# nfurnon/disco

Measured on NVIDIA H100. Metric: beamformed frames/sec (16kHz, 512-pt STFT), higher is better.
Workload: dtype f32 (c64 spectra, f32 SCM accumulation, f64 per-bin solve)

## Files before the change

### disco_b200/_lib.py

```python
import ctypes
import os

_HERE = os.path.dirname(os.path.abspath(__file__))
LIB_PATH = os.path.join(_HERE, "libdisco_b200.so")

c_int, c_void_p, c_size_t, c_float, c_double = (ctypes.c_int, ctypes.c_void_p, ctypes.c_size_t,
                                                ctypes.c_float, ctypes.c_double)
c_int_p = ctypes.POINTER(ctypes.c_int)

SIGNATURES = {
    "disco_abi_version": (c_int, []),
    "disco_last_error": (ctypes.c_char_p, []),
    "disco_n_frames": (c_int, [c_int, c_int]),
    "disco_init": (c_int, [c_int]),
    "disco_set_reserved_sms": (c_int, [c_int]),
    "disco_stft": (c_int, [c_void_p, c_void_p, c_int, c_int, c_int, c_void_p]),
    "disco_stft_scm_workspace": (c_size_t, [c_int, c_int, c_int, c_int]),
    "disco_stft_scm": (c_int, [c_void_p, c_void_p, c_int, c_void_p, c_void_p, c_void_p, c_int, c_int, c_int, c_int,
                               c_void_p, c_size_t, c_void_p]),
    "disco_stft_scm_supported": (c_int, [c_int, c_int, c_int]),
    "disco_stft_scm2_workspace": (c_size_t, [c_int, c_int, c_int, c_int]),
    "disco_stft_scm2": (c_int, [c_void_p, c_void_p, c_void_p, c_int, c_void_p, c_int, c_int, c_int, c_int, c_void_p,
                                c_size_t, c_void_p]),
    "disco_stft_filter_dual": (c_int, [c_void_p, c_void_p, c_void_p, c_void_p, c_void_p, c_void_p, c_int, c_int, c_int,
                                       c_int, c_int, c_int, c_void_p]),
    "disco_scm_from_workspace": (c_int, [c_void_p, c_int, c_int, c_void_p, c_void_p, c_int, c_int, c_int, c_int,
                                         c_void_p]),
    "disco_mwf_solve_workspace2": (c_int, [c_void_p, c_void_p, c_void_p, c_int, c_int, c_int, c_int, c_int, c_int,
                                           c_double, c_void_p]),
    "disco_filter_dual": (c_int, [c_void_p, c_void_p, c_void_p, c_void_p, c_void_p, c_void_p, c_int, c_int, c_int,
                                  c_int, c_int, c_int, c_void_p]),
    "disco_tf_mask": (c_int, [c_void_p, c_void_p, c_void_p, c_size_t, c_int, c_int, c_float, c_void_p]),
    "disco_masked_scm": (c_int, [c_void_p, c_void_p, c_void_p, c_int, c_void_p, c_void_p, c_int, c_int, c_int, c_int,
                                 c_int, c_int_p, c_int, c_int, c_void_p]),
    "disco_filter_sum_scm": (c_int, [c_void_p, c_void_p, c_void_p, c_int, c_void_p, c_void_p, c_int, c_void_p, c_void_p,
                                     c_int, c_int, c_int, c_int, c_void_p]),
    "disco_tango_mid_supported": (c_int, [c_int, c_int]),
    "disco_tango_mid": (c_int, [c_void_p, c_void_p, c_void_p, c_void_p, c_void_p, c_int, c_void_p, c_void_p, c_int, c_int,
                                c_int, c_int, c_int, c_void_p]),
    "disco_mwf_solve_workspace": (c_int, [c_void_p, c_void_p, c_void_p, c_void_p, c_void_p, c_int, c_int, c_int, c_int,
                                          c_int, c_int, c_double, c_void_p]),
    "disco_mwf_solve": (c_int, [c_void_p, c_void_p, c_void_p, c_void_p, c_int, c_int, c_int, c_int, c_double,
                                c_void_p]),
    "disco_filter_sum": (c_int, [c_void_p, c_int, c_void_p, c_void_p, c_void_p, c_void_p, c_int, c_int, c_int, c_int,
                                 c_int, c_int, c_int, c_int_p, c_int, c_int, c_void_p]),
    "disco_istft": (c_int, [c_void_p, c_void_p, c_int, c_int, c_int, c_int, c_void_p]),
    "disco_scm_recursive": (c_int, [c_void_p, c_void_p, c_void_p, c_void_p, c_void_p, c_void_p, c_void_p, ctypes.c_double,
                                    c_int, c_int, c_int, c_int, c_int, c_int, c_int, c_int_p, c_int, c_void_p]),
    "disco_filter_sum_blocks": (c_int, [c_void_p, c_int, c_void_p, c_void_p, c_void_p, c_void_p, c_int, c_int, c_int,
                                        c_int, c_int, c_int, c_int, c_int, c_int_p, c_int, c_void_p]),
    "disco_band_stats": (c_int, [c_void_p, c_void_p, c_void_p, c_void_p, c_int, c_int, ctypes.c_longlong, c_int, c_int,
                                 c_void_p]),
    "disco_transpose_c64": (c_int, [c_void_p, c_void_p, c_int, c_int, c_int, c_void_p]),
    "disco_transpose_f32": (c_int, [c_void_p, c_void_p, c_int, c_int, c_int, c_void_p]),
    "disco_apply_mask": (c_int, [c_void_p, c_void_p, c_void_p, c_size_t, c_int, c_void_p]),
    "disco_apply_mask_channels": (c_int, [c_void_p, c_void_p, c_void_p, c_size_t, c_int, c_size_t, c_int, c_void_p]),
}

_lib = None


def load():
    global _lib
    if _lib is not None:
        return _lib
    if not os.path.exists(LIB_PATH):
        raise ImportError(
            "disco_b200: %s not found -- build the CUDA library first (python -m disco_b200.build). "
            "There is no CPU or PyTorch fallback." % LIB_PATH)
    lib = ctypes.CDLL(LIB_PATH)
    for name, (res, args) in SIGNATURES.items():
        fn = getattr(lib, name)
        fn.restype = res
        fn.argtypes = args
    if lib.disco_abi_version() != 2:
        raise ImportError("disco_b200: ABI version mismatch")
    _lib = lib
    return lib


class DiscoError(RuntimeError):
    pass


def check(rc):
    if rc != 0:
        msg = load().disco_last_error()
        raise DiscoError("libdisco_b200 error %d: %s" % (rc, msg.decode() if msg else "?"))
```

### disco_b200/build.py

```python
import os
import subprocess
import sys
from concurrent.futures import ThreadPoolExecutor

HERE = os.path.dirname(os.path.abspath(__file__))
ROOT = os.path.dirname(HERE)
CSRC = os.path.join(HERE, "csrc")
OBJ = os.path.join(ROOT, "build", "obj")
LIB = os.path.join(HERE, "libdisco_b200.so")
SOURCES = ["api.cu", "stft_scm.cu", "scm.cu", "scm_wide.cu", "solve.cu", "solve_small.cu", "filter_sum.cu", "filter_sum_multi.cu", "filter_dual.cu", "mid_multi.cu", "istft.cu", "filterbank.cu", "online.cu", "misc.cu"]
NVCC = os.environ.get("NVCC", "/usr/local/cuda/bin/nvcc")
FLAGS = ["-O3", "-std=c++17", "-gencode", "arch=compute_90a,code=sm_90a", "-lineinfo",
         "-Xcompiler", "-fPIC", "-Xcompiler", "-fvisibility=hidden"]


def _deps_mtime():
    newest = 0.0
    for dirpath in (CSRC, os.path.join(ROOT, "include")):
        for fn in os.listdir(dirpath):
            if fn.endswith((".cuh", ".h")):
                newest = max(newest, os.path.getmtime(os.path.join(dirpath, fn)))
    return newest


def build(verbose=False, force=False):
    os.makedirs(OBJ, exist_ok=True)
    hdr = _deps_mtime()
    jobs = []
    for src in SOURCES:
        s = os.path.join(CSRC, src)
        o = os.path.join(OBJ, src.replace(".cu", ".o"))
        if force or not os.path.exists(o) or os.path.getmtime(o) < max(os.path.getmtime(s), hdr):
            cmd = [NVCC] + FLAGS + (["-Xptxas", "-v"] if verbose else []) + ["-c", s, "-o", o]
            jobs.append(cmd)

    def run(cmd):
        r = subprocess.run(cmd, capture_output=True, text=True)
        return cmd, r

    with ThreadPoolExecutor(max_workers=min(8, max(1, len(jobs)))) as ex:
        for cmd, r in ex.map(run, jobs):
            if verbose or r.returncode != 0:
                sys.stderr.write(" ".join(cmd) + "\n" + r.stdout + r.stderr + "\n")
            if r.returncode != 0:
                raise RuntimeError("nvcc failed for %s" % cmd[-3])
    objs = [os.path.join(OBJ, s.replace(".cu", ".o")) for s in SOURCES]
    if force or jobs or not os.path.exists(LIB):
        cmd = [NVCC, "-shared", "-o", LIB] + objs + ["-gencode", "arch=compute_90a,code=sm_90a"]
        r = subprocess.run(cmd, capture_output=True, text=True)
        if r.returncode != 0:
            sys.stderr.write(r.stdout + r.stderr)
            raise RuntimeError("link failed")
    return LIB


if __name__ == "__main__":
    print(build(verbose="-v" in sys.argv, force="--force" in sys.argv))
```

### disco_b200/csrc/stft_scm.cu

```cuda
#include "common.cuh"
#include "fft_reg.cuh"
#include "kernels.h"

namespace disco {

enum : int { OUT_Y = 0, OUT_NONE = 1, OUT_FILTER = 2, OUT_FILTER_FT = 3 };

template <int N, int C, int NM = 1, int OUT = OUT_Y>
struct StftCfg {
    static constexpr int RA = N / 32;
    static constexpr int NB = 32 / RA;
    static constexpr int HALF = N / 2;
    static constexpr int F = N / 2 + 1;
    static constexpr bool WIDE = C > 4;
    static constexpr int NSTG = 2;
    static constexpr int JOBS = 8;
    static constexpr int ITEMS = JOBS * NB;
    static constexpr int P = (C + 1) / 2;
    static constexpr int TT = ITEMS / P;
    static constexpr bool REALLOC = (N == 512) || (WIDE && N == 256);
    static constexpr int FFT_WARPS = (N == 512 && (WIDE || NM == 2)) ? 4 : 8;
    static constexpr int JPW = JOBS / FFT_WARPS;
    static constexpr int ROWP = 1056 / NB;
    static constexpr int SCM_WARPS = N / 64;
    static constexpr int LEAD_WARPS = REALLOC ? 4 : 1;
    static constexpr int WARPS = LEAD_WARPS + FFT_WARPS + SCM_WARPS;
    static constexpr int THREADS = 32 * WARPS;
    static constexpr int SPEC = ITEMS * ROWP;
    static constexpr int SAMP = C * (TT + 1) * HALF;
    static constexpr int REG_LAUNCH = 16384 / ((WARPS + 3) / 4) / 32 / 8 * 8;
    static constexpr bool FILT = OUT == OUT_FILTER || OUT == OUT_FILTER_FT;
    static constexpr int REG_LEAD = FILT ? 56 : 32;
    static constexpr int REG_SCM = FILT ? 80 : WIDE ? 184 : (FFT_WARPS == 4 ? 152 : 120);
    static constexpr int REG_FFT_CAP = 256;
    static constexpr int REG_ALLOC = (REG_LAUNCH > 255 ? 255 : REG_LAUNCH) * THREADS;
    static constexpr int REG_FFT_LEFT = (REG_ALLOC - 128 * REG_LEAD - 32 * SCM_WARPS * REG_SCM) / (32 * FFT_WARPS) / 8 * 8;
    static constexpr int REG_FFT = REG_FFT_LEFT < REG_FFT_CAP ? REG_FFT_LEFT : REG_FFT_CAP;
    static constexpr int REG_SUM = 128 * REG_LEAD + 32 * FFT_WARPS * REG_FFT + 32 * SCM_WARPS * REG_SCM;
    static constexpr int FT_PITCH = 34;
    static constexpr int FT_STAGE = OUT == OUT_FILTER_FT ? SCM_WARPS * 8 * FT_PITCH : 0;
    static_assert(!REALLOC || (REG_LEAD >= 24 && REG_FFT >= 24), "setmaxnreg budgets start at 24");
    static_assert(!REALLOC || REG_SUM <= (REG_LAUNCH > 255 ? 255 : REG_LAUNCH) * THREADS,
                  "register budgets exceed the CTA's allocation");
};

int stft_tile_frames(int n_fft, int C) { return (8 * (32 / (n_fft / 32))) / ((C + 1) / 2); }

template <int N, int C, int OUT = OUT_Y>
__host__ __device__ inline size_t smem_bytes() {
    using G = StftCfg<N, C, 1, OUT>;
    return G::NSTG * ((size_t)G::SPEC * sizeof(float2) + (size_t)G::SAMP * sizeof(float)) + (size_t)N * sizeof(float2) + 256 +
           64 * sizeof(float) + (size_t)G::FT_STAGE * sizeof(float2);
}

__device__ __forceinline__ long long range_lo(long long total, int b, int nb) { return total * b / nb; }

template <int R, int LAUNCH>
DISCO_DEV void set_maxnreg() {
    if constexpr (R > LAUNCH) {
        asm volatile("setmaxnreg.inc.sync.aligned.u32 %0;\n" ::"n"(R));
    } else if constexpr (R < LAUNCH) {
        asm volatile("setmaxnreg.dec.sync.aligned.u32 %0;\n" ::"n"(R));
    }
}

template <int C, int NM>
struct ScmAcc {
    static constexpr int NOFF = C * (C - 1) / 2;
    static constexpr int NO = NOFF > 0 ? NOFF : 1;
    float2 d[NM > 0 ? NM : 1][C];
    float2 os[NM > 0 ? NM : 1][NO];
    float2 on[NM > 0 ? NM : 1][NO];
    DISCO_DEV void reset() {
#pragma unroll
        for (int q = 0; q < NM; ++q) {
#pragma unroll
            for (int i = 0; i < C; ++i) d[q][i] = make_float2(0.f, 0.f);
#pragma unroll
            for (int i = 0; i < NOFF; ++i) os[q][i] = on[q][i] = make_float2(0.f, 0.f);
        }
    }
    DISCO_DEV void step(const float2 (&y)[C], const float (&m)[NM > 0 ? NM : 1]) {
        float2 ab[NM > 0 ? NM : 1];
#pragma unroll
        for (int q = 0; q < NM; ++q) {
            const float om = 1.f - m[q];
            ab[q] = make_float2(m[q] * m[q], om * om);
        }
        int o = 0;
#pragma unroll
        for (int i = 0; i < C; ++i) {
            const float dd = fmaf(y[i].x, y[i].x, y[i].y * y[i].y);
#pragma unroll
            for (int q = 0; q < NM; ++q) d[q][i] = ffma2(make_float2(dd, dd), ab[q], d[q][i]);
#pragma unroll
            for (int j = i + 1; j < C; ++j) {
                const float2 op = cmulc(y[i], y[j]);
#pragma unroll
                for (int q = 0; q < NM; ++q) {
                    os[q][o] = cfma_r(ab[q].x, op, os[q][o]);
                    on[q][o] = cfma_r(ab[q].y, op, on[q][o]);
                }
                ++o;
            }
        }
    }
    DISCO_DEV void flush(float* out, int F) const {
        int a = 0;
#pragma unroll
        for (int q = 0; q < NM; ++q) {
#pragma unroll
            for (int i = 0; i < C; ++i) out[(size_t)(a++) * F] = d[q][i].x;
#pragma unroll
            for (int i = 0; i < NOFF; ++i) {
                out[(size_t)(a++) * F] = os[q][i].x;
                out[(size_t)(a++) * F] = os[q][i].y;
            }
#pragma unroll
            for (int i = 0; i < C; ++i) out[(size_t)(a++) * F] = d[q][i].y;
#pragma unroll
            for (int i = 0; i < NOFF; ++i) {
                out[(size_t)(a++) * F] = on[q][i].x;
                out[(size_t)(a++) * F] = on[q][i].y;
            }
        }
    }
};

template <int OUT>
struct StftParam {
    using type = StftArgs;
};
template <>
struct StftParam<OUT_FILTER> {
    using type = StftFilterArgs;
};
template <>
struct StftParam<OUT_FILTER_FT> {
    using type = StftFilterArgs;
};

template <int N, int C, int NM, int OUT>
__global__ void __launch_bounds__(StftCfg<N, C, NM, OUT>::THREADS, 1) stft_scm_kernel(typename StftParam<OUT>::type p) {
    using G = StftCfg<N, C, NM, OUT>;
    constexpr int RA = G::RA, NB = G::NB, H = G::HALF, F = G::F, ROWP = G::ROWP, P = G::P, TT = G::TT;
    constexpr int SAMP = G::SAMP;
    constexpr int NACC = NM * 2 * C * C;
    constexpr int NMX = NM > 0 ? NM : 1;
    constexpr bool SCM = NM > 0;
    constexpr bool STORE_Y = OUT == OUT_Y, FILT = G::FILT, FT = OUT == OUT_FILTER_FT;
    static_assert(!FILT || NM == 0, "the filter consumer accumulates no statistics");
    constexpr int MCAP = (G::REALLOC && G::REG_SCM >= 152 && !G::WIDE) ? 16 : 8;
    constexpr int MC = (TT * NM <= MCAP) ? TT : ((MCAP / NMX) < TT ? (MCAP / NMX) : TT);
    constexpr int NCH = (TT + MC - 1) / MC;

    extern __shared__ __align__(128) unsigned char smem_raw[];
    constexpr int NSTG = G::NSTG;
    float2* spec = reinterpret_cast<float2*>(smem_raw);
    float* samp = reinterpret_cast<float*>(spec + NSTG * G::SPEC);
    float2* tw = reinterpret_cast<float2*>(samp + NSTG * SAMP);
    uint64_t* bars = reinterpret_cast<uint64_t*>(tw + N);
    uint64_t* samp_full = bars;
    uint64_t* samp_empty = bars + NSTG;
    uint64_t* spec_full = bars + 2 * NSTG;
    uint64_t* spec_empty = bars + 3 * NSTG;
    float* nyq = reinterpret_cast<float*>(bars + 32);
    float2* ft_stage = reinterpret_cast<float2*>(nyq + 64);
    static_assert(4 * NSTG <= 32, "barrier area");
    static_assert(TT * C <= 64 && TT <= 32, "Nyquist staging");

    const int tid = threadIdx.x, lane = tid & 31, warp = tid >> 5;
    const int L = p.L, T = p.T;
    const int tiles_per_grp = (T + TT - 1) / TT;
    const long long total = (long long)p.n_grp * tiles_per_grp;
    const long long lo = range_lo(total, blockIdx.x, gridDim.x), hi = range_lo(total, blockIdx.x + 1, gridDim.x);
    const int n_it = (int)(hi - lo);
    if (n_it <= 0) return;

    for (int i = tid; i < N; i += blockDim.x) tw[i] = p.twiddle[i];
    if (tid == 0) {
        for (int s = 0; s < NSTG; ++s) {
            mbar_init(&samp_full[s], 1);
            mbar_init(&samp_empty[s], G::FFT_WARPS);
            mbar_init(&spec_full[s], G::FFT_WARPS);
            mbar_init(&spec_empty[s], G::SCM_WARPS + 1);
        }
        fence_mbar_init();
    }
    __syncthreads();

    auto tile_of = [&](int it, int& grp, int& t0) {
        const long long i = lo + it;
        grp = (int)(i / tiles_per_grp);
        t0 = (int)(i % tiles_per_grp) * TT;
    };
    auto seg_slot = [&](int grp) { return blockIdx.x - seg_slots(grp, tiles_per_grp, total, gridDim.x).first; };
    auto mask_at = [&](int q, int grp, int t, int f) {
        const float* m = q == 0 ? p.mask : p.mask2;
        return p.mask_ft ? m[((size_t)grp * F + f) * T + t] : m[((size_t)grp * T + t) * F + f];
    };

    constexpr int FFT_WARP0 = G::LEAD_WARPS;
    constexpr int SCM_WARP0 = G::LEAD_WARPS + G::FFT_WARPS;
    const bool is_fft = warp >= FFT_WARP0 && warp < FFT_WARP0 + G::FFT_WARPS;
    if (warp < G::LEAD_WARPS) {
        if (G::REALLOC) set_maxnreg<G::REG_LEAD, G::REG_LAUNCH>();
        if (warp != 0) return;
        auto load_tile = [&](int it) {
            int grp, t0;
            tile_of(it, grp, t0);
            const int nfr = min(TT, T - t0), s = it % NSTG, c_valid = min(C, p.n_sig - grp * C);
            mbar_wait(&samp_empty[s], ((it / NSTG) & 1) ^ 1);
            const float* xg = p.x + (size_t)grp * C * L;
            float* dst = samp + s * SAMP;
            const int s0 = t0 * H - H;
            const int cnt = (nfr + 1) * H;
            const int k_lo = max(0, -s0), k_hi = min(cnt, L - s0);
            if (lane == 0) {
                if (p.use_tma && k_hi > k_lo) {
                    fence_proxy_async();
                    mbar_expect_tx(&samp_full[s], (uint32_t)(c_valid * (k_hi - k_lo) * sizeof(float)));
                    for (int c = 0; c < c_valid; ++c)
                        tma_load_1d(dst + c * (TT + 1) * H + k_lo, xg + (size_t)c * L + s0 + k_lo,
                                    (uint32_t)((k_hi - k_lo) * sizeof(float)), &samp_full[s]);
                } else {
                    mbar_arrive(&samp_full[s]);
                }
            }
        };
        constexpr int NP = C * (C + 1) / 2;
        constexpr int NSLOT = NP > 32 ? 2 : 1;
        int pi[NSLOT], pj[NSLOT], row[NSLOT];
#pragma unroll
        for (int u = 0; u < NSLOT; ++u) {
            const int pp = min(lane + 32 * u, NP - 1);
            if (pp < C) {
                pi[u] = pj[u] = pp;
                row[u] = pp;
            } else {
                int o = pp - C, i = 0, n = C - 1;
                while (o >= n) {
                    o -= n;
                    --n;
                    ++i;
                }
                pi[u] = i;
                pj[u] = i + 1 + o;
                row[u] = C + 2 * (pp - C);
            }
        }
        float as[NMX][NSLOT], an[NMX][NSLOT];
        auto nyq_reset = [&]() {
#pragma unroll
            for (int q = 0; q < NMX; ++q)
#pragma unroll
                for (int u = 0; u < NSLOT; ++u) as[q][u] = an[q][u] = 0.f;
        };
        nyq_reset();
        float2 nw1[FILT ? C : 1], nw2[FILT ? C : 1];
        int nw_grp = -1;
        for (int i = 0; i < NSTG - 1; ++i)
            if (i < n_it) load_tile(i);
        for (int it = 0; it < n_it; ++it) {
            if (it + NSTG - 1 < n_it) load_tile(it + NSTG - 1);
            int grp, t0;
            tile_of(it, grp, t0);
            const int nfr = min(TT, T - t0), s = it % NSTG, c_valid = min(C, p.n_sig - grp * C);
            if constexpr (FILT) {
                if (grp != nw_grp) {
#pragma unroll
                    for (int c = 0; c < C; ++c) {
                        nw1[c] = p.W1[((size_t)grp * F + F - 1) * C + c];
                        nw2[c] = p.W2[((size_t)grp * F + F - 1) * C + c];
                    }
                    nw_grp = grp;
                }
                mbar_wait(&spec_full[s], (it / NSTG) & 1);
                if (lane < nfr) {
                    float2 y[C];
#pragma unroll
                    for (int c = 0; c < C; ++c) {
                        const float2 z = spec[s * G::SPEC + (size_t)(lane * P + c / 2) * ROWP + N / 2];
                        y[c] = make_float2((c & 1) ? z.y + z.y : z.x + z.x, 0.f);
                    }
                    float2 z, zn, yf;
                    dual_filter<C>(nw1, nw2, y, p.ref, z, zn, yf);
                    const size_t o = FT ? ((size_t)grp * F + F - 1) * T + t0 + lane : ((size_t)grp * T + t0 + lane) * F + (F - 1);
                    __stcs(p.z + o, z);
                    if (p.zn) __stcs(p.zn + o, zn);
                    __stcs(p.yf + o, yf);
                }
                __syncwarp();
                if (lane == 0) mbar_arrive(&spec_empty[s]);
            } else {
                float mq[NMX];
#pragma unroll
                for (int q = 0; q < NMX; ++q) mq[q] = (SCM && lane < nfr) ? mask_at(q, grp, t0 + lane, F - 1) : 0.f;
                mbar_wait(&spec_full[s], (it / NSTG) & 1);
#pragma unroll
                for (int r = lane; r < TT * C; r += 32) {
                    const int tl_l = r / C, c_l = r % C;
                    float yv = 0.f;
                    if (tl_l < nfr && c_l < c_valid) {
                        const float2 z = spec[s * G::SPEC + (size_t)(tl_l * P + c_l / 2) * ROWP + N / 2];
                        yv = (c_l & 1) ? z.y + z.y : z.x + z.x;
                        if (STORE_Y) p.Y[(((size_t)grp * C + c_l) * T + t0 + tl_l) * F + (F - 1)] = make_float2(yv, 0.f);
                    }
                    nyq[r] = yv;
                }
                __syncwarp();
                if (lane == 0) mbar_arrive(&spec_empty[s]);
                if (SCM) {
#pragma unroll
                    for (int tl = 0; tl < TT; ++tl) {
                        if (tl < nfr) {
                            float pr[NSLOT];
#pragma unroll
                            for (int u = 0; u < NSLOT; ++u)
                                pr[u] = nyq[tl * C + pi[u]] * nyq[tl * C + pj[u]];
#pragma unroll
                            for (int q = 0; q < NM; ++q) {
                                const float m = __shfl_sync(0xffffffffu, mq[q], tl), om = 1.f - m;
                                const float a = m * m, b = om * om;
#pragma unroll
                                for (int u = 0; u < NSLOT; ++u) {
                                    as[q][u] = fmaf(a, pr[u], as[q][u]);
                                    an[q][u] = fmaf(b, pr[u], an[q][u]);
                                }
                            }
                        }
                    }
                    const bool seg_end = (it + 1 == n_it) || ((lo + it + 1) % tiles_per_grp == 0);
                    if (seg_end) {
                        float* out = p.part + ((size_t)grp * p.slots_per_grp + seg_slot(grp)) * NACC * F + (F - 1);
#pragma unroll
                        for (int u = 0; u < NSLOT; ++u) {
                            const int pp = lane + 32 * u;
                            if (pp < NP) {
#pragma unroll
                                for (int q = 0; q < NM; ++q) {
                                    float* os = out + (size_t)(q * 2 * C * C) * F;
                                    float* on = os + (size_t)(C * C) * F;
                                    os[(size_t)row[u] * F] = as[q][u];
                                    on[(size_t)row[u] * F] = an[q][u];
                                    if (pp >= C) {
                                        os[(size_t)(row[u] + 1) * F] = 0.f;
                                        on[(size_t)(row[u] + 1) * F] = 0.f;
                                    }
                                }
                            }
                        }
                        nyq_reset();
                    }
                }
                __syncwarp();
            }
        }
    } else if (is_fft) {
        if (G::REALLOC) set_maxnreg<G::REG_FFT, G::REG_LAUNCH>();
        const int wf = warp - FFT_WARP0, f0 = wf / G::FFT_WARPS, w = wf % G::FFT_WARPS;
        constexpr bool WINREG = (RA <= 16);
        float win[WINREG ? RA : 1];
        if (WINREG) {
#pragma unroll
            for (int j = 0; j < RA; ++j) win[j] = p.window[lane + 32 * j];
        }
        for (int it = f0; it < n_it; ++it) {
            int grp, t0;
            tile_of(it, grp, t0);
            const int nfr = min(TT, T - t0), s = it % NSTG, c_valid = min(C, p.n_sig - grp * C);
            const uint32_t ph = (it / NSTG) & 1;
            const float* sm = samp + s * SAMP;
            mbar_wait(&samp_full[s], ph);
            {
                const int s0 = t0 * H - H;
                const int cnt = (nfr + 1) * H;
                int k_lo = max(0, -s0), k_hi = min(cnt, L - s0);
                if (!p.use_tma || k_hi <= k_lo) k_lo = k_hi = 0;
                const int n_fill = cnt - (k_hi - k_lo);
                if (n_fill > 0) {
                    const float* xg = p.x + (size_t)grp * C * L;
                    float* dst = samp + s * SAMP;
                    named_bar_sync(1 + f0, 32 * G::FFT_WARPS);
                    for (int c = 0; c < c_valid; ++c)
#pragma unroll 4
                        for (int q = w * 32 + lane; q < n_fill; q += 32 * G::FFT_WARPS) {
                            const int k = q < k_lo ? q : q + (k_hi - k_lo);
                            int sidx = s0 + k;
                            if (sidx < 0) sidx = -sidx;
                            if (sidx >= L) sidx = 2 * (L - 1) - sidx;
                            float v = 0.f;
                            if (sidx >= 0 && sidx < L) v = xg[(size_t)c * L + sidx];
                            dst[c * (TT + 1) * H + k] = v;
                        }
                    named_bar_sync(1 + f0, 32 * G::FFT_WARPS);
                }
            }
            mbar_wait(&spec_empty[s], ph ^ 1);
            const bool full = (nfr == TT && c_valid == C && (C % 2 == 0) && (G::ITEMS % P == 0));
#pragma unroll 1
            for (int jj = 0; jj < G::JPW; ++jj) {
                const int jb = w * G::JPW + jj;
                float2* job = spec + s * G::SPEC + (size_t)jb * NB * ROWP;
                constexpr bool TWREG = (RA <= 16);
                float2 twr[TWREG ? RA : 1];
                if (TWREG) {
#pragma unroll
                    for (int k1 = 1; k1 < RA; ++k1) twr[k1] = tw[k1 * 32 + lane];
                }
#pragma unroll
                for (int q = 0; q < NB; ++q) {
                    const int item = jb * NB + q;
                    const int tl = item / P, pr = item % P;
                    const int ca = 2 * pr, cb = 2 * pr + 1;
                    const float* xa = sm + ca * (TT + 1) * H + tl * H + lane;
                    const float* xb = sm + cb * (TT + 1) * H + tl * H + lane;
                    float2 v[RA];
                    if (full || (tl < nfr && cb < c_valid)) {
#pragma unroll
                        for (int j = 0; j < RA; ++j) {
                            const float wj = WINREG ? win[j] : p.window[lane + 32 * j];
                            v[j] = fmul2(make_float2(xa[32 * j], xb[32 * j]), make_float2(wj, wj));
                        }
                    } else if (tl < nfr && ca < c_valid) {
#pragma unroll
                        for (int j = 0; j < RA; ++j) {
                            const float wj = WINREG ? win[j] : p.window[lane + 32 * j];
                            v[j] = make_float2(xa[32 * j] * wj, 0.f);
                        }
                    } else {
#pragma unroll
                        for (int j = 0; j < RA; ++j) v[j] = make_float2(0.f, 0.f);
                    }
                    if (jj == G::JPW - 1 && q == NB - 1) {
                        __syncwarp();
                        if (lane == 0) mbar_arrive(&samp_empty[s]);
                    }
                    dft_reg<RA, false>(v);
#pragma unroll
                    for (int k1 = 1; k1 < RA; ++k1) v[k1] = cmul(v[k1], TWREG ? twr[k1] : tw[k1 * 32 + lane]);
#pragma unroll
                    for (int k1 = 0; k1 < RA; ++k1) job[(q * RA + k1) * 33 + lane] = v[k1];
                }
                __syncwarp();
                float2 u[32];
#pragma unroll
                for (int l = 0; l < 32; ++l) u[l] = job[lane * 33 + l];
                __syncwarp();
                dft_reg<32, false>(u);
                {
                    float2* row = job + (lane / RA) * ROWP + (lane % RA);
#pragma unroll
                    for (int k2 = 0; k2 < 32; ++k2) row[RA * k2] = u[k2];
                }
            }
            __syncwarp();
            if (lane == 0) mbar_arrive(&spec_full[s]);
        }
    } else {
        if (G::REALLOC) set_maxnreg<G::REG_SCM, G::REG_LAUNCH>();
        const int f = (warp - SCM_WARP0) * 32 + lane;
        const int fn = (N - f) & (N - 1);
        if constexpr (FILT) {
            float2 w1[C], w2[C];
            int w_grp = -1;
            for (int it = 0; it < n_it; ++it) {
                int grp, t0;
                tile_of(it, grp, t0);
                const int nfr = min(TT, T - t0), s = it % NSTG;
                if (grp != w_grp) {
#pragma unroll
                    for (int c = 0; c < C; ++c) {
                        w1[c] = p.W1[((size_t)grp * F + f) * C + c];
                        w2[c] = p.W2[((size_t)grp * F + f) * C + c];
                    }
                    w_grp = grp;
                }
                const float2* stage = spec + s * G::SPEC;
                auto point = [&](int tl, float2& z, float2& zn, float2& yf) {
                    float2 y[C];
#pragma unroll
                    for (int pr = 0; pr < P; ++pr) {
                        const float2* row = stage + (size_t)(tl * P + pr) * ROWP;
                        const float2 zf = row[f], zb = row[fn];
                        y[2 * pr] = fadd2(zf, make_float2(zb.x, -zb.y));
                        if (2 * pr + 1 < C) y[2 * pr + 1] = fadd2(make_float2(zf.y, -zf.x), make_float2(zb.y, zb.x));
                    }
                    dual_filter<C>(w1, w2, y, p.ref, z, zn, yf);
                };
                mbar_wait(&spec_full[s], (it / NSTG) & 1);
                if constexpr (!FT) {
                    const size_t o = ((size_t)grp * T + t0) * F + f;
#pragma unroll 8
                    for (int tl = 0; tl < TT; ++tl) {
                        if (tl < nfr) {
                            float2 z, zn, yf;
                            point(tl, z, zn, yf);
                            __stcs(p.z + o + (size_t)tl * F, z);
                            if (p.zn) __stcs(p.zn + o + (size_t)tl * F, zn);
                            __stcs(p.yf + o + (size_t)tl * F, yf);
                        }
                    }
                } else {
                    float2* st = ft_stage + (warp - SCM_WARP0) * 8 * G::FT_PITCH;
                    const int fw = (warp - SCM_WARP0) * 32, jl = lane & 7;
                    auto flush = [&](float2* out, int c8) {
                        __syncwarp();
                        if (c8 + jl < nfr) {
#pragma unroll
                            for (int k = 0; k < 8; ++k) {
                                const int i = (lane >> 3) + 4 * k;
                                __stcs(out + ((size_t)grp * F + fw + i) * T + t0 + c8 + jl, st[jl * G::FT_PITCH + i]);
                            }
                        }
                        __syncwarp();
                    };
#pragma unroll 1
                    for (int c8 = 0; c8 < nfr; c8 += 8) {
                        float2 znr[8], yfr[8];
#pragma unroll
                        for (int j = 0; j < 8; ++j) {
                            float2 z = make_float2(0.f, 0.f);
                            znr[j] = yfr[j] = z;
                            if (c8 + j < nfr) point(c8 + j, z, znr[j], yfr[j]);
                            st[j * G::FT_PITCH + lane] = z;
                        }
                        flush(p.z, c8);
                        if (p.zn) {
#pragma unroll
                            for (int j = 0; j < 8; ++j) st[j * G::FT_PITCH + lane] = znr[j];
                            flush(p.zn, c8);
                        }
#pragma unroll
                        for (int j = 0; j < 8; ++j) st[j * G::FT_PITCH + lane] = yfr[j];
                        flush(p.yf, c8);
                    }
                }
                __syncwarp();
                if (lane == 0) mbar_arrive(&spec_empty[s]);
            }
            return;
        }
        ScmAcc<C, NM> acc;
        float mk[NMX][MC];
        const int m_st = p.mask_ft ? 1 : F;
        const size_t m_f = p.mask_ft ? (size_t)f * T : (size_t)f;
        auto load_mask = [&](int it, int ch) {
            if (it >= n_it) return;
            int grp, t0;
            tile_of(it, grp, t0);
            const size_t base = (size_t)grp * T * F + m_f + (size_t)(t0 + ch * MC) * m_st;
#pragma unroll
            for (int q = 0; q < NM; ++q) {
                const float* mb = (q == 0 ? p.mask : p.mask2) + base;
#pragma unroll
                for (int i = 0; i < MC; ++i)
                    mk[q][i] = (ch * MC + i < TT && t0 + ch * MC + i < T) ? mb[i * m_st] : 0.f;
            }
        };
        if (SCM) {
            acc.reset();
            load_mask(0, 0);
        }
        for (int it = 0; it < n_it; ++it) {
            int grp, t0;
            tile_of(it, grp, t0);
            const int nfr = min(TT, T - t0), s = it % NSTG, c_valid = min(C, p.n_sig - grp * C);
            const float2* stage = spec + s * G::SPEC;
            float2* ybase = p.Y + ((size_t)grp * C * T + t0) * F + f;
            const size_t cstride = (size_t)T * F;
            const bool full = (nfr == TT && c_valid == C);
#pragma unroll
            for (int ch = 0; ch < NCH; ++ch) {
                float mcur[NMX][MC];
#pragma unroll
                for (int q = 0; q < NMX; ++q)
#pragma unroll
                    for (int i = 0; i < MC; ++i) mcur[q][i] = SCM ? mk[q][i] : 0.f;
                if (SCM) {
                    if (ch + 1 < NCH)
                        load_mask(it, ch + 1);
                    else
                        load_mask(it + 1, 0);
                }
                if (ch == 0) mbar_wait(&spec_full[s], (it / NSTG) & 1);
#pragma unroll
                for (int i = 0; i < MC; ++i) {
                    const int tl = ch * MC + i;
                    if (tl < TT && (full || tl < nfr)) {
                        float2 y[C];
#pragma unroll
                        for (int pr = 0; pr < P; ++pr) {
                            const float2* row = stage + (size_t)(tl * P + pr) * ROWP;
                            const float2 zf = row[f], zn = row[fn];
                            y[2 * pr] = fadd2(zf, make_float2(zn.x, -zn.y));
                            if (2 * pr + 1 < C) y[2 * pr + 1] = fadd2(make_float2(zf.y, -zf.x), make_float2(zn.y, zn.x));
                        }
                        if (STORE_Y) {
#pragma unroll
                            for (int c = 0; c < C; ++c)
                                if (full || c < c_valid) __stcs(ybase + c * cstride + tl * F, y[c]);
                        }
                        if (SCM) {
                            float m[NMX];
#pragma unroll
                            for (int q = 0; q < NMX; ++q) m[q] = mcur[q][i];
                            acc.step(y, m);
                        }
                    }
                }
            }
            __syncwarp();
            if (lane == 0) mbar_arrive(&spec_empty[s]);
            const bool seg_end = (it + 1 == n_it) || ((lo + it + 1) % tiles_per_grp == 0);
            if (SCM && seg_end) {
                acc.flush(p.part + ((size_t)grp * p.slots_per_grp + seg_slot(grp)) * NACC * F + f, F);
                acc.reset();
            }
        }
    }
}

template <int C>
__global__ void __launch_bounds__(288) scm_finalize_kernel(const float* __restrict__ part, float2* __restrict__ Rss,
                                                           float2* __restrict__ Rnn, int n_grp, int slots_per_grp,
                                                           int tiles_per_grp, int n_cta, int F, float inv_T, int n_set,
                                                           int set) {
    constexpr int NA = 2 * C * C;
    const int g = blockIdx.x;
    const long long total = (long long)n_grp * tiles_per_grp;
    const int n_slot = seg_slots(g, tiles_per_grp, total, n_cta).count();
    const size_t slot_stride = (size_t)n_set * NA * F;
    for (int f = threadIdx.x; f < F; f += blockDim.x) {
        const float* base = part + (size_t)g * slots_per_grp * slot_stride + (size_t)set * NA * F + f;
#pragma unroll 1
        for (int which = 0; which < 2; ++which) {
            float acc[C * C];
#pragma unroll
            for (int a = 0; a < C * C; ++a) acc[a] = 0.f;
            for (int sl = 0; sl < n_slot; ++sl) {
#pragma unroll
                for (int a = 0; a < C * C; ++a) acc[a] += __ldg(base + sl * slot_stride + (size_t)(which * C * C + a) * F);
            }
            float2* R = (which == 0 ? Rss : Rnn) + ((size_t)g * F + f) * C * C;
            int o = 0;
#pragma unroll
            for (int i = 0; i < C; ++i) {
                R[i * C + i] = make_float2(acc[i] * inv_T, 0.f);
#pragma unroll
                for (int j = i + 1; j < C; ++j) {
                    const float re = acc[C + 2 * o] * inv_T, im = acc[C + 2 * o + 1] * inv_T;
                    R[i * C + j] = make_float2(re, im);
                    R[j * C + i] = make_float2(re, -im);
                    ++o;
                }
            }
        }
    }
}

int stft_tiles_per_grp(int n_fft, int C, int T) {
    const int tt = stft_tile_frames(n_fft, C);
    return (T + tt - 1) / tt;
}

bool stft_scm_supported(int n_fft, int C, int n_mask) {
    if (C < 1 || C > 8 || n_mask < 0 || n_mask > 2) return false;
    if (n_fft != 256 && n_fft != 512 && n_fft != 1024) return false;
    if (C > 4 && (n_mask == 2 || n_fft == 1024)) return false;
    if (n_mask == 2 && n_fft == 1024) return false;
    if (n_mask == 0 && C > 4) return false;
    return true;
}

template <int N, int C, int NM, int OUT = OUT_Y>
static cudaError_t launch_one(const typename StftParam<OUT>::type& a, int n_cta, cudaStream_t st) {
    using G = StftCfg<N, C, NM, OUT>;
    auto kern = stft_scm_kernel<N, C, NM, OUT>;
    const size_t smem = smem_bytes<N, C, OUT>();
    cudaError_t e = cudaFuncSetAttribute(kern, cudaFuncAttributeMaxDynamicSharedMemorySize, (int)smem);
    if (e != cudaSuccess) return e;
    if (G::REALLOC) {
        cudaFuncAttributes fa;
        e = cudaFuncGetAttributes(&fa, kern);
        if (e != cudaSuccess) return e;
        if ((long long)fa.numRegs * G::THREADS < G::REG_SUM) return cudaErrorLaunchOutOfResources;
    }
    kern<<<n_cta, G::THREADS, smem, st>>>(a);
    return cudaGetLastError();
}

template <int N, int C>
static cudaError_t launch_nm(const StftArgs& a, int nm, int n_cta, cudaStream_t st) {
    if constexpr (C <= 4) {
        if (nm == 0) return launch_one<N, C, 0>(a, n_cta, st);
    }
    if (nm == 1) return launch_one<N, C, 1>(a, n_cta, st);
    if constexpr (C <= 4 && N <= 512) {
        if (nm == 2) return a.Y ? launch_one<N, C, 2>(a, n_cta, st) : launch_one<N, C, 2, OUT_NONE>(a, n_cta, st);
    }
    return cudaErrorInvalidValue;
}

template <int N>
static cudaError_t launch_c(const StftArgs& a, int C, int nm, int n_cta, cudaStream_t st) {
    switch (C) {
        case 1: return launch_nm<N, 1>(a, nm, n_cta, st);
        case 2: return launch_nm<N, 2>(a, nm, n_cta, st);
        case 3: return launch_nm<N, 3>(a, nm, n_cta, st);
        case 4: return launch_nm<N, 4>(a, nm, n_cta, st);
        default: break;
    }
    if constexpr (N <= 512) {
        switch (C) {
            case 5: return launch_nm<N, 5>(a, nm, n_cta, st);
            case 6: return launch_nm<N, 6>(a, nm, n_cta, st);
            case 7: return launch_nm<N, 7>(a, nm, n_cta, st);
            case 8: return launch_nm<N, 8>(a, nm, n_cta, st);
            default: break;
        }
    }
    return cudaErrorInvalidValue;
}

cudaError_t launch_stft_scm(const StftArgs& a, int n_fft, int C, int n_cta, int n_mask, cudaStream_t st) {
    if (!stft_scm_supported(n_fft, C, n_mask)) return cudaErrorInvalidValue;
    switch (n_fft) {
        case 256: return launch_c<256>(a, C, n_mask, n_cta, st);
        case 512: return launch_c<512>(a, C, n_mask, n_cta, st);
        case 1024: return launch_c<1024>(a, C, n_mask, n_cta, st);
        default: return cudaErrorInvalidValue;
    }
}

cudaError_t launch_stft_filter_dual(const StftFilterArgs& a, int n_fft, int C, int n_cta, cudaStream_t st) {
    if (!stft_scm_supported(n_fft, C, 2)) return cudaErrorInvalidValue;
#define DISCO_SFD(NN, CC)                                                                                  \
    if (n_fft == NN && C == CC)                                                                            \
        return a.out_ft ? launch_one<NN, CC, 0, OUT_FILTER_FT>(a, n_cta, st) : launch_one<NN, CC, 0, OUT_FILTER>(a, n_cta, st);
    DISCO_SFD(256, 1) DISCO_SFD(256, 2) DISCO_SFD(256, 3) DISCO_SFD(256, 4)
    DISCO_SFD(512, 1) DISCO_SFD(512, 2) DISCO_SFD(512, 3) DISCO_SFD(512, 4)
#undef DISCO_SFD
    return cudaErrorInvalidValue;
}

cudaError_t launch_scm_finalize(const float* part, float2* Rss, float2* Rnn, int n_grp, int slots_per_grp,
                                int tiles_per_grp, int n_cta, int C, int F, int T, int n_set, int set, cudaStream_t st) {
    const float inv_T = 1.0f / (float)T;
#define DISCO_FIN(CC)                                                                                              \
    case CC:                                                                                                       \
        scm_finalize_kernel<CC><<<n_grp, 288, 0, st>>>(part, Rss, Rnn, n_grp, slots_per_grp, tiles_per_grp, n_cta, \
                                                       F, inv_T, n_set, set);                                      \
        break;
    switch (C) {
        DISCO_FIN(1)
        DISCO_FIN(2)
        DISCO_FIN(3)
        DISCO_FIN(4)
        DISCO_FIN(5)
        DISCO_FIN(6)
        DISCO_FIN(7)
        DISCO_FIN(8)
        default: return cudaErrorInvalidValue;
    }
#undef DISCO_FIN
    return cudaGetLastError();
}

}
```

Baseline: 94.46 million.

## Deal FFT jobs round-robin across seven warps for two-mask 512-point configs

For 512-point STFT with two masks and three or more microphones, the producer split changes: the three idle lead warps are dropped and seven FFT warps take jobs round-robin across tiles. Every job now arrives on the fill and spectrum barriers, and the registers from the lead and FFT warps are pooled at 104 each next to the SCM warps. The aim is to raise FFT throughput by using more warps instead of four warps at high register counts, at the cost of per-job barrier arrivals and fewer registers per FFT warp. The change also adds optional per-role clock instrumentation and build options for defines and an alternate library path.

```diff
diff --git a/disco_b200/_lib.py b/disco_b200/_lib.py
--- a/disco_b200/_lib.py
+++ b/disco_b200/_lib.py
@@ -2,7 +2,7 @@
 import os
 
 _HERE = os.path.dirname(os.path.abspath(__file__))
-LIB_PATH = os.path.join(_HERE, "libdisco_b200.so")
+LIB_PATH = os.environ.get("DISCO_B200_LIB") or os.path.join(_HERE, "libdisco_b200.so")
 
 c_int, c_void_p, c_size_t, c_float, c_double = (ctypes.c_int, ctypes.c_void_p, ctypes.c_size_t,
                                                 ctypes.c_float, ctypes.c_double)
diff --git a/disco_b200/build.py b/disco_b200/build.py
--- a/disco_b200/build.py
+++ b/disco_b200/build.py
@@ -23,15 +23,16 @@
     return newest
 
 
-def build(verbose=False, force=False):
-    os.makedirs(OBJ, exist_ok=True)
+def build(verbose=False, force=False, defines=(), lib=LIB, obj=OBJ):
+    os.makedirs(obj, exist_ok=True)
     hdr = _deps_mtime()
     jobs = []
     for src in SOURCES:
         s = os.path.join(CSRC, src)
-        o = os.path.join(OBJ, src.replace(".cu", ".o"))
+        o = os.path.join(obj, src.replace(".cu", ".o"))
         if force or not os.path.exists(o) or os.path.getmtime(o) < max(os.path.getmtime(s), hdr):
-            cmd = [NVCC] + FLAGS + (["-Xptxas", "-v"] if verbose else []) + ["-c", s, "-o", o]
+            cmd = ([NVCC] + FLAGS + ["-D" + d for d in defines] + (["-Xptxas", "-v"] if verbose else []) +
+                   ["-c", s, "-o", o])
             jobs.append(cmd)
 
     def run(cmd):
@@ -44,14 +45,14 @@
                 sys.stderr.write(" ".join(cmd) + "\n" + r.stdout + r.stderr + "\n")
             if r.returncode != 0:
                 raise RuntimeError("nvcc failed for %s" % cmd[-3])
-    objs = [os.path.join(OBJ, s.replace(".cu", ".o")) for s in SOURCES]
-    if force or jobs or not os.path.exists(LIB):
-        cmd = [NVCC, "-shared", "-o", LIB] + objs + ["-gencode", "arch=compute_90a,code=sm_90a"]
+    objs = [os.path.join(obj, s.replace(".cu", ".o")) for s in SOURCES]
+    if force or jobs or not os.path.exists(lib):
+        cmd = [NVCC, "-shared", "-o", lib] + objs + ["-gencode", "arch=compute_90a,code=sm_90a"]
         r = subprocess.run(cmd, capture_output=True, text=True)
         if r.returncode != 0:
             sys.stderr.write(r.stdout + r.stderr)
             raise RuntimeError("link failed")
-    return LIB
+    return lib
 
 
 if __name__ == "__main__":
diff --git a/disco_b200/csrc/stft_scm.cu b/disco_b200/csrc/stft_scm.cu
--- a/disco_b200/csrc/stft_scm.cu
+++ b/disco_b200/csrc/stft_scm.cu
@@ -19,29 +19,41 @@
     static constexpr int P = (C + 1) / 2;
     static constexpr int TT = ITEMS / P;
     static constexpr bool REALLOC = (N == 512) || (WIDE && N == 256);
-    static constexpr int FFT_WARPS = (N == 512 && (WIDE || NM == 2)) ? 4 : 8;
+    static constexpr bool DEAL = N == 512 && NM == 2 && C >= 3 && !WIDE;
+    static constexpr int FFT_WARPS = DEAL ? 7 : (N == 512 && (WIDE || NM == 2)) ? 4 : 8;
     static constexpr int JPW = JOBS / FFT_WARPS;
+    static constexpr int FFT_ARRIVALS = DEAL ? JOBS : FFT_WARPS;
     static constexpr int ROWP = 1056 / NB;
     static constexpr int SCM_WARPS = N / 64;
-    static constexpr int LEAD_WARPS = REALLOC ? 4 : 1;
+    static constexpr int LEAD_WARPS = (REALLOC && !DEAL) ? 4 : 1;
     static constexpr int WARPS = LEAD_WARPS + FFT_WARPS + SCM_WARPS;
     static constexpr int THREADS = 32 * WARPS;
     static constexpr int SPEC = ITEMS * ROWP;
     static constexpr int SAMP = C * (TT + 1) * HALF;
     static constexpr int REG_LAUNCH = 16384 / ((WARPS + 3) / 4) / 32 / 8 * 8;
     static constexpr bool FILT = OUT == OUT_FILTER || OUT == OUT_FILTER_FT;
-    static constexpr int REG_LEAD = FILT ? 56 : 32;
-    static constexpr int REG_SCM = FILT ? 80 : WIDE ? 184 : (FFT_WARPS == 4 ? 152 : 120);
+    static constexpr int REG_SCM = FILT ? 80 : WIDE ? 184 : ((N == 512 && NM == 2) ? 152 : 120);
     static constexpr int REG_FFT_CAP = 256;
     static constexpr int REG_ALLOC = (REG_LAUNCH > 255 ? 255 : REG_LAUNCH) * THREADS;
-    static constexpr int REG_FFT_LEFT = (REG_ALLOC - 128 * REG_LEAD - 32 * SCM_WARPS * REG_SCM) / (32 * FFT_WARPS) / 8 * 8;
+    static constexpr int REG_LEAD_OWN = FILT ? 56 : 32;
+    static constexpr int REG_FFT_LEFT =
+        DEAL ? (REG_ALLOC - 32 * SCM_WARPS * REG_SCM) / (32 * (LEAD_WARPS + FFT_WARPS)) / 8 * 8
+             : (REG_ALLOC - 128 * REG_LEAD_OWN - 32 * SCM_WARPS * REG_SCM) / (32 * FFT_WARPS) / 8 * 8;
     static constexpr int REG_FFT = REG_FFT_LEFT < REG_FFT_CAP ? REG_FFT_LEFT : REG_FFT_CAP;
-    static constexpr int REG_SUM = 128 * REG_LEAD + 32 * FFT_WARPS * REG_FFT + 32 * SCM_WARPS * REG_SCM;
+    static constexpr int REG_LEAD = DEAL ? REG_FFT : REG_LEAD_OWN;
+    static constexpr int REG_SUM = DEAL ? 32 * (LEAD_WARPS + FFT_WARPS) * REG_FFT + 32 * SCM_WARPS * REG_SCM
+                                        : 128 * REG_LEAD + 32 * FFT_WARPS * REG_FFT + 32 * SCM_WARPS * REG_SCM;
     static constexpr int FT_PITCH = 34;
     static constexpr int FT_STAGE = OUT == OUT_FILTER_FT ? SCM_WARPS * 8 * FT_PITCH : 0;
     static_assert(!REALLOC || (REG_LEAD >= 24 && REG_FFT >= 24), "setmaxnreg budgets start at 24");
     static_assert(!REALLOC || REG_SUM <= (REG_LAUNCH > 255 ? 255 : REG_LAUNCH) * THREADS,
                   "register budgets exceed the CTA's allocation");
+    static_assert(!DEAL || (REALLOC && LEAD_WARPS + FFT_WARPS == 8 && WARPS == 16 && REG_LAUNCH == 128 &&
+                            REG_FFT == 104 && REG_SUM == 65536),
+                  "DEAL: loader + 7 FFT warps fill two warpgroups at 104 registers next to 8 SCM warps at 152");
+    static_assert(DEAL || WIDE || NM != 2 || N != 512 || (FFT_WARPS == 4 && REG_SCM == 152 && REG_FFT == 176),
+                  "two masks, 1-2 microphones at 512 points: 4 FFT warps at 176 registers next to SCM warps at 152");
+    static_assert(!DEAL || JOBS >= FFT_WARPS, "DEAL: every FFT warp must run a job of every tile (the fill barrier)");
 };
 
 int stft_tile_frames(int n_fft, int C) { return (8 * (32 / (n_fft / 32))) / ((C + 1) / 2); }
@@ -126,6 +138,47 @@
         }
     }
 };
+
+enum : int { RC_SAMP_FULL = 0, RC_SAMP_EMPTY = 1, RC_SPEC_FULL = 2, RC_SPEC_EMPTY = 3 };
+enum : int { RC_ROLE_LOADER = 1, RC_ROLE_FFT = 2, RC_ROLE_SCM = 3 };
+#ifdef DISCO_ROLE_CLOCKS
+constexpr int RC_MAX_CTAS = 1024, RC_SLOTS = 8;
+__device__ unsigned long long g_role_clocks[RC_MAX_CTAS * 32 * RC_SLOTS];
+DISCO_DEV long long rc_clock() {
+    long long t;
+    asm volatile("mov.u64 %0, %%clock64;" : "=l"(t)::"memory");
+    return t;
+}
+struct RoleClocks {
+    long long t0, w[4] = {0, 0, 0, 0};
+    int tiles = 0, jobs = 0;
+    DISCO_DEV RoleClocks() : t0(rc_clock()) {}
+    DISCO_DEV void wait(int k, uint64_t* bar, uint32_t parity) {
+        const long long a = rc_clock();
+        mbar_wait(bar, parity);
+        w[k] += rc_clock() - a;
+    }
+    DISCO_DEV void tile() { ++tiles; }
+    DISCO_DEV void job() { ++jobs; }
+    DISCO_DEV void done(int role) {
+        const long long t1 = rc_clock();
+        if ((threadIdx.x & 31) != 0 || blockIdx.x >= RC_MAX_CTAS) return;
+        unsigned long long* o = g_role_clocks + ((size_t)blockIdx.x * 32 + (threadIdx.x >> 5)) * RC_SLOTS;
+        o[0] = role;
+        o[1] = tiles;
+        o[2] = jobs;
+        o[3] = t1 - t0;
+        for (int k = 0; k < 4; ++k) o[4 + k] = w[k];
+    }
+};
+#else
+struct RoleClocks {
+    DISCO_DEV void wait(int, uint64_t* bar, uint32_t parity) { mbar_wait(bar, parity); }
+    DISCO_DEV void tile() {}
+    DISCO_DEV void job() {}
+    DISCO_DEV void done(int) {}
+};
+#endif
 
 template <int OUT>
 struct StftParam {
@@ -181,8 +234,8 @@
     if (tid == 0) {
         for (int s = 0; s < NSTG; ++s) {
             mbar_init(&samp_full[s], 1);
-            mbar_init(&samp_empty[s], G::FFT_WARPS);
-            mbar_init(&spec_full[s], G::FFT_WARPS);
+            mbar_init(&samp_empty[s], G::FFT_ARRIVALS);
+            mbar_init(&spec_full[s], G::FFT_ARRIVALS);
             mbar_init(&spec_empty[s], G::SCM_WARPS + 1);
         }
         fence_mbar_init();
@@ -203,14 +256,18 @@
     constexpr int FFT_WARP0 = G::LEAD_WARPS;
     constexpr int SCM_WARP0 = G::LEAD_WARPS + G::FFT_WARPS;
     const bool is_fft = warp >= FFT_WARP0 && warp < FFT_WARP0 + G::FFT_WARPS;
+    if constexpr (G::DEAL) {
+        if (warp < SCM_WARP0) set_maxnreg<G::REG_FFT, G::REG_LAUNCH>();
+    }
     if (warp < G::LEAD_WARPS) {
-        if (G::REALLOC) set_maxnreg<G::REG_LEAD, G::REG_LAUNCH>();
+        if (G::REALLOC && !G::DEAL) set_maxnreg<G::REG_LEAD, G::REG_LAUNCH>();
         if (warp != 0) return;
+        RoleClocks rc;
         auto load_tile = [&](int it) {
             int grp, t0;
             tile_of(it, grp, t0);
             const int nfr = min(TT, T - t0), s = it % NSTG, c_valid = min(C, p.n_sig - grp * C);
-            mbar_wait(&samp_empty[s], ((it / NSTG) & 1) ^ 1);
+            rc.wait(RC_SAMP_EMPTY, &samp_empty[s], ((it / NSTG) & 1) ^ 1);
             const float* xg = p.x + (size_t)grp * C * L;
             float* dst = samp + s * SAMP;
             const int s0 = t0 * H - H;
@@ -275,7 +332,7 @@
                     }
                     nw_grp = grp;
                 }
-                mbar_wait(&spec_full[s], (it / NSTG) & 1);
+                rc.wait(RC_SPEC_FULL, &spec_full[s], (it / NSTG) & 1);
                 if (lane < nfr) {
                     float2 y[C];
 #pragma unroll
@@ -296,7 +353,7 @@
                 float mq[NMX];
 #pragma unroll
                 for (int q = 0; q < NMX; ++q) mq[q] = (SCM && lane < nfr) ? mask_at(q, grp, t0 + lane, F - 1) : 0.f;
-                mbar_wait(&spec_full[s], (it / NSTG) & 1);
+                rc.wait(RC_SPEC_FULL, &spec_full[s], (it / NSTG) & 1);
 #pragma unroll
                 for (int r = lane; r < TT * C; r += 32) {
                     const int tl_l = r / C, c_l = r % C;
@@ -355,9 +412,11 @@
                 }
                 __syncwarp();
             }
-        }
+            rc.tile();
+        }
+        rc.done(RC_ROLE_LOADER);
     } else if (is_fft) {
-        if (G::REALLOC) set_maxnreg<G::REG_FFT, G::REG_LAUNCH>();
+        if (G::REALLOC && !G::DEAL) set_maxnreg<G::REG_FFT, G::REG_LAUNCH>();
         const int wf = warp - FFT_WARP0, f0 = wf / G::FFT_WARPS, w = wf % G::FFT_WARPS;
         constexpr bool WINREG = (RA <= 16);
         float win[WINREG ? RA : 1];
@@ -365,13 +424,19 @@
 #pragma unroll
             for (int j = 0; j < RA; ++j) win[j] = p.window[lane + 32 * j];
         }
-        for (int it = f0; it < n_it; ++it) {
+        RoleClocks rc;
+        struct FftTile {
+            int s, nfr, c_valid;
+            const float* sm;
+            bool full;
+        };
+        auto enter_tile = [&](int it) {
             int grp, t0;
             tile_of(it, grp, t0);
             const int nfr = min(TT, T - t0), s = it % NSTG, c_valid = min(C, p.n_sig - grp * C);
             const uint32_t ph = (it / NSTG) & 1;
             const float* sm = samp + s * SAMP;
-            mbar_wait(&samp_full[s], ph);
+            rc.wait(RC_SAMP_FULL, &samp_full[s], ph);
             {
                 const int s0 = t0 * H - H;
                 const int cnt = (nfr + 1) * H;
@@ -383,7 +448,7 @@
                     float* dst = samp + s * SAMP;
                     named_bar_sync(1 + f0, 32 * G::FFT_WARPS);
                     for (int c = 0; c < c_valid; ++c)
-#pragma unroll 4
+#pragma unroll(G::DEAL ? 1 : 4)
                         for (int q = w * 32 + lane; q < n_fill; q += 32 * G::FFT_WARPS) {
                             const int k = q < k_lo ? q : q + (k_hi - k_lo);
                             int sidx = s0 + k;
@@ -396,71 +461,99 @@
                     named_bar_sync(1 + f0, 32 * G::FFT_WARPS);
                 }
             }
-            mbar_wait(&spec_empty[s], ph ^ 1);
+            rc.wait(RC_SPEC_EMPTY, &spec_empty[s], ph ^ 1);
             const bool full = (nfr == TT && c_valid == C && (C % 2 == 0) && (G::ITEMS % P == 0));
+            return FftTile{s, nfr, c_valid, sm, full};
+        };
+        auto run_job = [&](const FftTile& tc, int jb, bool release) {
+            const int s = tc.s, nfr = tc.nfr, c_valid = tc.c_valid;
+            const float* sm = tc.sm;
+            const bool full = tc.full;
+            float2* job = spec + s * G::SPEC + (size_t)jb * NB * ROWP;
+            constexpr bool TWREG = (RA <= 16);
+            float2 twr[TWREG ? RA : 1];
+            if (TWREG) {
+#pragma unroll
+                for (int k1 = 1; k1 < RA; ++k1) twr[k1] = tw[k1 * 32 + lane];
+            }
+#pragma unroll
+            for (int q = 0; q < NB; ++q) {
+                const int item = jb * NB + q;
+                const int tl = item / P, pr = item % P;
+                const int ca = 2 * pr, cb = 2 * pr + 1;
+                const float* xa = sm + ca * (TT + 1) * H + tl * H + lane;
+                const float* xb = sm + cb * (TT + 1) * H + tl * H + lane;
+                float2 v[RA];
+                if (full || (tl < nfr && cb < c_valid)) {
+#pragma unroll
+                    for (int j = 0; j < RA; ++j) {
+                        const float wj = WINREG ? win[j] : p.window[lane + 32 * j];
+                        v[j] = fmul2(make_float2(xa[32 * j], xb[32 * j]), make_float2(wj, wj));
+                    }
+                } else if (tl < nfr && ca < c_valid) {
+#pragma unroll
+                    for (int j = 0; j < RA; ++j) {
+                        const float wj = WINREG ? win[j] : p.window[lane + 32 * j];
+                        v[j] = make_float2(xa[32 * j] * wj, 0.f);
+                    }
+                } else {
+#pragma unroll
+                    for (int j = 0; j < RA; ++j) v[j] = make_float2(0.f, 0.f);
+                }
+                if (release && q == NB - 1) {
+                    __syncwarp();
+                    if (lane == 0) mbar_arrive(&samp_empty[s]);
+                }
+                dft_reg<RA, false>(v);
+#pragma unroll
+                for (int k1 = 1; k1 < RA; ++k1) v[k1] = cmul(v[k1], TWREG ? twr[k1] : tw[k1 * 32 + lane]);
+#pragma unroll
+                for (int k1 = 0; k1 < RA; ++k1) job[(q * RA + k1) * 33 + lane] = v[k1];
+            }
+            __syncwarp();
+            float2 u[32];
+#pragma unroll
+            for (int l = 0; l < 32; ++l) u[l] = job[lane * 33 + l];
+            __syncwarp();
+            dft_reg<32, false>(u);
+            {
+                float2* row = job + (lane / RA) * ROWP + (lane % RA);
+#pragma unroll
+                for (int k2 = 0; k2 < 32; ++k2) row[RA * k2] = u[k2];
+            }
+            rc.job();
+        };
+        if constexpr (G::DEAL) {
+            FftTile tc{};
+            int cur = -1;
 #pragma unroll 1
-            for (int jj = 0; jj < G::JPW; ++jj) {
-                const int jb = w * G::JPW + jj;
-                float2* job = spec + s * G::SPEC + (size_t)jb * NB * ROWP;
-                constexpr bool TWREG = (RA <= 16);
-                float2 twr[TWREG ? RA : 1];
-                if (TWREG) {
-#pragma unroll
-                    for (int k1 = 1; k1 < RA; ++k1) twr[k1] = tw[k1 * 32 + lane];
-                }
-#pragma unroll
-                for (int q = 0; q < NB; ++q) {
-                    const int item = jb * NB + q;
-                    const int tl = item / P, pr = item % P;
-                    const int ca = 2 * pr, cb = 2 * pr + 1;
-                    const float* xa = sm + ca * (TT + 1) * H + tl * H + lane;
-                    const float* xb = sm + cb * (TT + 1) * H + tl * H + lane;
-                    float2 v[RA];
-                    if (full || (tl < nfr && cb < c_valid)) {
-#pragma unroll
-                        for (int j = 0; j < RA; ++j) {
-                            const float wj = WINREG ? win[j] : p.window[lane + 32 * j];
-                            v[j] = fmul2(make_float2(xa[32 * j], xb[32 * j]), make_float2(wj, wj));
-                        }
-                    } else if (tl < nfr && ca < c_valid) {
-#pragma unroll
-                        for (int j = 0; j < RA; ++j) {
-                            const float wj = WINREG ? win[j] : p.window[lane + 32 * j];
-                            v[j] = make_float2(xa[32 * j] * wj, 0.f);
-                        }
-                    } else {
-#pragma unroll
-                        for (int j = 0; j < RA; ++j) v[j] = make_float2(0.f, 0.f);
-                    }
-                    if (jj == G::JPW - 1 && q == NB - 1) {
-                        __syncwarp();
-                        if (lane == 0) mbar_arrive(&samp_empty[s]);
-                    }
-                    dft_reg<RA, false>(v);
-#pragma unroll
-                    for (int k1 = 1; k1 < RA; ++k1) v[k1] = cmul(v[k1], TWREG ? twr[k1] : tw[k1 * 32 + lane]);
-#pragma unroll
-                    for (int k1 = 0; k1 < RA; ++k1) job[(q * RA + k1) * 33 + lane] = v[k1];
-                }
+            for (int j = w; j < n_it * G::JOBS; j += G::FFT_WARPS) {
+                const int it = j / G::JOBS;
+                if (it != cur) {
+                    tc = enter_tile(it);
+                    cur = it;
+                    rc.tile();
+                }
+                run_job(tc, j % G::JOBS, true);
                 __syncwarp();
-                float2 u[32];
-#pragma unroll
-                for (int l = 0; l < 32; ++l) u[l] = job[lane * 33 + l];
+                if (lane == 0) mbar_arrive(&spec_full[tc.s]);
+            }
+        } else {
+            for (int it = f0; it < n_it; ++it) {
+                const FftTile tc = enter_tile(it);
+#pragma unroll 1
+                for (int jj = 0; jj < G::JPW; ++jj) run_job(tc, w * G::JPW + jj, jj == G::JPW - 1);
                 __syncwarp();
-                dft_reg<32, false>(u);
-                {
-                    float2* row = job + (lane / RA) * ROWP + (lane % RA);
-#pragma unroll
-                    for (int k2 = 0; k2 < 32; ++k2) row[RA * k2] = u[k2];
-                }
-            }
-            __syncwarp();
-            if (lane == 0) mbar_arrive(&spec_full[s]);
-        }
+                if (lane == 0) mbar_arrive(&spec_full[tc.s]);
+                rc.tile();
+            }
+        }
+        rc.done(RC_ROLE_FFT);
     } else {
         if (G::REALLOC) set_maxnreg<G::REG_SCM, G::REG_LAUNCH>();
         const int f = (warp - SCM_WARP0) * 32 + lane;
         const int fn = (N - f) & (N - 1);
+        RoleClocks rc;
         if constexpr (FILT) {
             float2 w1[C], w2[C];
             int w_grp = -1;
@@ -488,7 +581,7 @@
                     }
                     dual_filter<C>(w1, w2, y, p.ref, z, zn, yf);
                 };
-                mbar_wait(&spec_full[s], (it / NSTG) & 1);
+                rc.wait(RC_SPEC_FULL, &spec_full[s], (it / NSTG) & 1);
                 if constexpr (!FT) {
                     const size_t o = ((size_t)grp * T + t0) * F + f;
 #pragma unroll 8
@@ -538,7 +631,9 @@
                 }
                 __syncwarp();
                 if (lane == 0) mbar_arrive(&spec_empty[s]);
-            }
+                rc.tile();
+            }
+            rc.done(RC_ROLE_SCM);
             return;
         }
         ScmAcc<C, NM> acc;
@@ -583,7 +678,7 @@
                     else
                         load_mask(it + 1, 0);
                 }
-                if (ch == 0) mbar_wait(&spec_full[s], (it / NSTG) & 1);
+                if (ch == 0) rc.wait(RC_SPEC_FULL, &spec_full[s], (it / NSTG) & 1);
 #pragma unroll
                 for (int i = 0; i < MC; ++i) {
                     const int tl = ch * MC + i;
@@ -617,7 +712,9 @@
                 acc.flush(p.part + ((size_t)grp * p.slots_per_grp + seg_slot(grp)) * NACC * F + f, F);
                 acc.reset();
             }
-        }
+            rc.tile();
+        }
+        rc.done(RC_ROLE_SCM);
     }
 }
 
@@ -768,3 +865,22 @@
 }
 
 }
+
+#ifdef DISCO_ROLE_CLOCKS
+extern "C" __attribute__((visibility("default"))) void disco_role_clocks_layout(int* max_ctas, int* slots) {
+    *max_ctas = disco::RC_MAX_CTAS;
+    *slots = disco::RC_SLOTS;
+}
+extern "C" __attribute__((visibility("default"))) long long disco_role_clocks(void* dst, size_t bytes, int reset) {
+    const size_t n = sizeof(disco::g_role_clocks) < bytes ? sizeof(disco::g_role_clocks) : bytes;
+    if (cudaDeviceSynchronize() != cudaSuccess) return -1;
+    if (n && cudaMemcpyFromSymbol(dst, disco::g_role_clocks, n) != cudaSuccess) return -1;
+    if (reset) {
+        void* a = nullptr;
+        if (cudaGetSymbolAddress(&a, disco::g_role_clocks) != cudaSuccess ||
+            cudaMemset(a, 0, sizeof(disco::g_role_clocks)) != cudaSuccess || cudaDeviceSynchronize() != cudaSuccess)
+            return -1;
+    }
+    return (long long)n;
+}
+#endif
```

Result: faster. 99.63 million, median of 6 (+5.5%).
